# amirhajibabaei/AutoForce

Hardware: AMD Instinct MI355X
Metric: MD-step atoms*steps/sec (SGPR predict: NL + descriptors + K_nm + E/F/stress + covloss); `value`: a Langevin MD loop on the device, every step from the forces of the one before (sgpr_md_run; --steps dependent steps between two fences); `value_resident_frames`: steps over independent frames resident i (higher is better)
Workload: dtype f64

## Files before the change

### autoforce_amd/csrc/api.hip

```cpp
#include <math.h>
#include <stdarg.h>
#include <stdio.h>
#include <stdlib.h>
#include <string.h>

#include <algorithm>
#include <numeric>

#include <dlfcn.h>
#include <unistd.h>
#include <rccl/rccl.h>

#include "../../include/sgpr_hip.h"
#include "sgpr_internal.h"
#include <cmath>
#include <limits>

static thread_local char g_err[512] = "";
static int fail(int code, const char *fmt, ...)
{
    va_list ap;
    va_start(ap, fmt);
    vsnprintf(g_err, sizeof(g_err), fmt, ap);
    va_end(ap);
// ... 341 lines not shown
        const int r = r0 + k, c = c0 + threadIdx.x;
        t[k][threadIdx.x] = (r < rows && c < cols) ? A[(size_t)r * lda + c] : 0.0;
    }
    __syncthreads();
    for (int k = threadIdx.y; k < 32; k += blockDim.y) {
        const int c = c0 + k, r = r0 + threadIdx.x;
        if (c < cols && r < rows) B[(size_t)c * ldb + r] = t[threadIdx.x][k];
    }
}

#define SGPR_MD_SCAL 16
struct FinNext {
    int mode;
    int S, cap, force, step;
    int pbc[3];
    double thr2;
    const double *pos_in;
    const int *iperm, *cslot;
    double *pos;
    int *flags;
    int *bc_next, *bc_cur;
    int *bin_of, *kslot;
    BinRec *b_rec;
    BinAux *b_aux;
    double *csq_rw;
    const double *x_cur, *v_cur;
    double *x_next, *v_next;
    const double *mass, *sig;
    const double *noise;
    unsigned long long seed;
    long long t_index;
    double hdt, c1;
    int nh, nh_first;
    const double *x_prev;
    double *v_now;
    const double *nh_zeta;
    int pending;
    double *ke_cur;
    const double *ke_prev, *packed_prev;
    double ediff;
    int *halt;
    int *halt_host;
    double *scal_cur, *scal_prev;
    int *mark_cur;
};

struct FinArgs {
    int N, cnt, first, stride, maxnn, t_stride, has_beta, nE, nV, bin_cap, t_check, csq_slots;
    int nbins_clear;
    const int *perm, *slot, *nn, *nbr_j, *aux, *nn_raw;
    const unsigned short *T;
    const double *G;
    const double *Fnbr, *Fself;
    const double *csq, *vs_sqrt, *Epart, *virpart;
    double mean_energy;
    double *packed;
    int *stat, *bin_count;
    const int *row_cols, *row_colslot, *nbr_code;
    size_t g_stride, f_stride, v_stride, p_stride;
    int xp;
    int xcmax;
    size_t scal_off;
    const int *flag;
    int *rebuilds;
    const double *pos;
    double *pos0;
    const double *cell;
    const NlGrid *grid;
    double *cell0;
    FinNext nx;
};

template <int CTRL>
__device__ __forceinline__ double fin_dpp(double v)
{
    const int lo = __builtin_amdgcn_update_dpp(0, __double2loint(v), CTRL, 0xf, 0xf, true);
    const int hi = __builtin_amdgcn_update_dpp(0, __double2hiint(v), CTRL, 0xf, 0xf, true);
    return __hiloint2double(hi, lo);
}
__device__ __forceinline__ double fin_lane(double v, int l)
{
    return __hiloint2double(__builtin_amdgcn_readlane(__double2hiint(v), l), __builtin_amdgcn_readlane(__double2loint(v), l));
}
__device__ __forceinline__ double fin_wave_sum(double v)
{
    v += fin_dpp<0xB1>(v);
    v += fin_dpp<0x4E>(v);
    v += fin_dpp<0x141>(v);
    v += fin_dpp<0x140>(v);
    return (fin_lane(v, 0) + fin_lane(v, 16)) + (fin_lane(v, 32) + fin_lane(v, 48));
}

__device__ __forceinline__ void finalize_reduce(const FinArgs &f, int q)
{
    __shared__ double wsum[4];
    const int tid = threadIdx.x, wave = tid >> 6, lane = tid & 63;
    const size_t by = blockIdx.y;
    double s = 0.0;
    if (q == 10) {
        int m8[8] = {0, 0, 0, 0, 0, 0, 0, 0};
        const int4 *src4 = (const int4 *)f.nn_raw;
        const int n4 = (f.cnt + 3) / 4;
        for (int k0 = tid; k0 < n4; k0 += 1024) {
#pragma unroll
            for (int u = 0; u < 4; u++) {
                const int k = k0 + 256 * u;
                const int4 v = src4[min(k, n4 - 1)];
                const int e = 4 * k;
                int m = e < f.cnt ? v.x : 0;
                m = max(m, e + 1 < f.cnt ? v.y : 0);
                m = max(m, e + 2 < f.cnt ? v.z : 0);
                m = max(m, e + 3 < f.cnt ? v.w : 0);
                m8[u] = max(m8[u], m);
            }
        }
        const int mx = max(max(max(m8[0], m8[1]), max(m8[2], m8[3])), max(max(m8[4], m8[5]), max(m8[6], m8[7])));
        s = (double)mx;
#pragma unroll
        for (int o = 32; o > 0; o >>= 1) s = fmax(s, __shfl_xor(s, o, 64));
    } else {
        const double *src = q == 0 ? f.Epart : f.virpart + by * f.v_stride + (size_t)(q - 1) * f.nV;
        const int n = q == 0 ? f.nE : f.nV;
        double a8[8] = {0.0, 0.0, 0.0, 0.0, 0.0, 0.0, 0.0, 0.0};
        for (int k0 = tid; k0 < n; k0 += 2048) {
#pragma unroll
            for (int u = 0; u < 8; u++) {
                const int k = k0 + 256 * u;
                const double v = src[min(k, n - 1)];
                a8[u] += k < n ? v : 0.0;
            }
        }
        s = ((a8[0] + a8[1]) + (a8[2] + a8[3])) + ((a8[4] + a8[5]) + (a8[6] + a8[7]));
        s = fin_wave_sum(s);
    }
    if (lane == 0) wsum[wave] = s;
    __syncthreads();
    if (tid == 0) {
        if (q == 10 && by == 0) {
            if (*f.flag) {
                atomicAdd(f.rebuilds, 1);
                if (f.cell0 && f.cell) {
                    double cv[18];
#pragma unroll
                    for (int k = 0; k < 9; k++) { cv[k] = f.cell[k]; cv[9 + k] = f.grid->inv[k]; }
#pragma unroll
                    for (int k = 0; k < 18; k++) f.cell0[k] = cv[k];
                }
            }
            const int mx = (int)fmax(fmax(wsum[0], wsum[1]), fmax(wsum[2], wsum[3]));
            f.stat[0] = max(f.stat[0], mx);
            const bool ov = mx > f.maxnn || f.stat[1] > f.bin_cap || (f.t_check && f.stat[2] > f.t_stride) || f.stat[3] != 0;
            f.packed[f.scal_off + 10] = ov ? 1.0 : 0.0;
            if (f.nx.mode == 2) {
                f.nx.scal_cur[10] = ov ? 1.0 : 0.0;
                *f.nx.mark_cur = 1;
                if (ov) {
                    atomicMin(&f.nx.halt[0], f.nx.step);
                    f.nx.halt_host[1] = f.nx.step;
                }
            }
        } else if (q != 10) {
            const double v = ((wsum[0] + wsum[1]) + (wsum[2] + wsum[3])) + (q == 0 ? f.mean_energy : 0.0);
            f.packed[by * f.p_stride + f.scal_off + q] = v;
            if (f.nx.mode == 2) f.nx.scal_cur[q] = v;
        }
    }
}

__device__ __forceinline__ void finalize_reduce_prev(const FinArgs &f, int q)
{
    __shared__ double wprev[4], wprev2[4];
    const int tid = threadIdx.x, wave = tid >> 6, lane = tid & 63;
    const int N = f.N;
// ... 232 lines not shown
    if (lane < 3) packed[3 * (size_t)c + lane] = fs - (lane == 0 ? fx : lane == 1 ? fy : fz);
    if (lane < 3 && *f.flag) f.pos0[3 * (size_t)i + lane] = f.pos[3 * (size_t)i + lane];
    if (lane == 3) {
        const double v = 1.0 - cs;
        packed[3 * (size_t)f.N + c] = f.has_beta ? sqrt(v > 0.0 ? v : 0.0) * vs : 0.0;
    }
}

__device__ __forceinline__ double md_deviate(unsigned long long seed, long long t, int atom, int comp)
{
    unsigned c0 = (unsigned)t, c1 = (unsigned)((unsigned long long)t >> 32), c2 = (unsigned)atom, c3 = (unsigned)comp;
    unsigned k0 = (unsigned)seed, k1 = (unsigned)(seed >> 32);
#pragma unroll
    for (int r = 0; r < 10; r++) {
        const unsigned long long p0 = (unsigned long long)0xD2511F53u * c0, p1 = (unsigned long long)0xCD9E8D57u * c2;
        const unsigned n0 = (unsigned)(p1 >> 32) ^ c1 ^ k0, n1 = (unsigned)p1, n2 = (unsigned)(p0 >> 32) ^ c3 ^ k1, n3 = (unsigned)p0;
        c0 = n0; c1 = n1; c2 = n2; c3 = n3;
        k0 += 0x9E3779B9u; k1 += 0xBB67AE85u;
    }
    const unsigned long long a = ((unsigned long long)c0 << 32) | c1, b = ((unsigned long long)c2 << 32) | c3;
    const double u1 = (double)((a >> 11) + 1ull) * (1.0 / 9007199254740992.0);
    const double u2 = (double)(b >> 11) * (1.0 / 9007199254740992.0);
    return sqrt(-2.0 * log(u1)) * cos(6.283185307179586 * u2);
}

__global__ void md_deviates_kernel(int N, int rows, unsigned long long seed, long long t0, double *out)
{
    const size_t n3 = (size_t)3 * N, tot = n3 * rows;
    for (size_t e = (size_t)blockIdx.x * blockDim.x + threadIdx.x; e < tot; e += (size_t)gridDim.x * blockDim.x) {
        const size_t r = e / n3, w = e - r * n3;
        out[e] = md_deviate(seed, t0 + (long long)r, (int)(w / 3), (int)(w % 3));
    }
}

__device__ __forceinline__ double md_nh_advance(const FinNext &x, double F, double ms, double xc, double v0, double xprev, double zeta, double &xn)
{
#pragma clang fp contract(off)
    const double dt = 2.0 * x.hdt;
    const double a = __ddiv_rn((dt * dt) * F, ms);
    double xp = xprev;
    if (x.nh_first) xp = (xc - dt * v0) + 0.5 * a;
    const double b = x.hdt * zeta;
    const double num = ((2.0 * xc) - xp * (1.0 - b)) + a;
    xn = __ddiv_rn(num, 1.0 + b);
    return x.nh_first ? v0 : __ddiv_rn(xn - xp, 2.0 * dt);
}

__global__ __launch_bounds__(256) void md_nh_kernel(int N, const double *ke, double *zeta, int n, double dt, double c1, double c2, double K0,
                                                    const int *halt, int step, double *scal_row)
{
    if (*halt < step) return;
    __shared__ double wsum[4];
    const int tid = threadIdx.x;
    double s = 0.0;
    for (int k = tid; k < N; k += 256) s += ke[2 * (size_t)k];
    s = fin_wave_sum(s);
    if ((tid & 63) == 0) wsum[tid >> 6] = s;
    __syncthreads();
    if (tid == 0) {
#pragma clang fp contract(off)
        const double KE = 0.5 * ((wsum[0] + wsum[1]) + (wsum[2] + wsum[3]));
        const int sc = n & 3, sn = (n + 1) & 3, sp = (n + 3) & 3;
        const double d = KE - K0;
        const double zprev = n == 0 ? -(c1 * d) : zeta[sp];
        const double zcur = n == 0 ? 0.0 : zeta[sc];
        const double zint = n == 0 ? 0.0 : zeta[4 + sc];
        const double znew = zprev + c2 * d;
        zeta[sn] = znew;
        zeta[4 + sn] = zint + dt * znew;
        scal_row[14] = zcur;
        scal_row[15] = zint;
    }
}

template <int MODE>
__global__ __launch_bounds__(256) void finalize_next_kernel(FinArgs f)
{
    const int tid = threadIdx.x, b = blockIdx.x, nA = gridDim.x - 13;
    const FinNext &x = f.nx;
    const int halt_w = MODE == 2 ? *x.halt : 0x7fffffff;
    if (b >= nA) {
        if (halt_w < x.step) return;
        if (b >= nA + 11) {
            if (MODE == 2 && x.packed_prev) finalize_reduce_prev(f, b - nA - 11);
        } else
            finalize_reduce(f, b - nA);
        return;
    }
    const int s1 = x.step + 1;
    const int wave = __builtin_amdgcn_readfirstlane(tid >> 6), lane = tid & 63;
    const int i = b * 4 + wave;
    const bool act = i < f.N;
    const int ia = act ? i : 0;
    const int l3 = lane < 3 ? lane : 2, lg = lane < f.maxnn ? lane : f.maxnn - 1, lc = lane < f.csq_slots ? lane : f.csq_slots - 1;
    const int rebuilt = *f.flag;
    const NlGrid g = *f.grid;
    const double2 *grow = (const double2 *)(f.G + ((size_t)ia * f.maxnn + lg) * 4);
    double2 g0 = grow[0], g1 = grow[1];
    const int n_ld = f.nn[ia];
    double fs = f.Fself[3 * (size_t)ia + l3];
    const int c = f.perm[ia];
    const int slot_i = f.slot[ia];
    const int ib = MODE == 1 ? x.iperm[ia] : ia;
    const int slot_b = MODE == 1 ? x.cslot[ia] : slot_i;
    double xc = 0.0, p0 = 0.0, vc = 0.0, ms = 1.0, sg = 0.0, nz = 0.0, xn = 0.0;
    if (MODE == 1) xn = x.pos_in[3 * (size_t)ia + l3];
    if (MODE == 2) {
        xc = x.x_cur[3 * (size_t)ia + l3];
        p0 = f.pos0[3 * (size_t)ia + l3];
        vc = x.v_cur[3 * (size_t)ia + l3];
        ms = x.mass[ia];
        sg = x.sig[ia];
        nz = x.noise ? x.noise[3 * (size_t)ia + l3] : 0.0;
    }
    double xpv = 0.0, zeta = 0.0;
    if (MODE == 2 && x.nh) { xpv = x.x_prev[3 * (size_t)ia + l3]; zeta = *x.nh_zeta; }
    double csv = f.has_beta ? f.csq[(size_t)ia * f.csq_slots + lc] : 0.0;
    if (lane >= f.csq_slots) csv = 0.0;
    if (f.has_beta)
        for (int k = lane + 64; k < f.csq_slots; k += 64) csv += f.csq[(size_t)ia * f.csq_slots + k];
    if (lane >= f.maxnn) { g0 = make_double2(0.0, 0.0); g1 = g0; }
    if (lane >= 3) fs = 0.0;
    const int n = act ? n_ld : 0;
    const double vs = f.has_beta ? f.vs_sqrt[slot_i < x.S ? slot_i : 0] : 0.0;
    if (MODE == 1) {
        xc = x.pos[3 * (size_t)ib + l3];
        p0 = f.pos0[3 * (size_t)ib + l3];
    }
    if (halt_w < x.step) return;
    for (int k = b * 256 + tid; k < f.nbins_clear; k += nA * 256) x.bc_cur[(size_t)k * SGPR_BIN_STRIDE] = 0;
    if (b == 0 && tid == 0) {
        if (x.force) atomicMax(&x.flags[s1 & 3], 1);
        x.flags[(s1 + 2) & 3] = 0;
        fin_cell_guard(f, rebuilt, s1);
    }
    if (!act) return;
    if (f.has_beta)
        for (int k = lane; k < f.csq_slots; k += 64) x.csq_rw[(size_t)i * f.csq_slots + k] = 0.0;
    int bin = 0, kb = -1, w0 = 0, w1 = 0, w2 = 0;
    auto place = [&](double X, double Y, double Z) {
        int bidx[3], w[3];
#pragma unroll
        for (int k = 0; k < 3; k++) {
            double fr = X * g.inv[k] + Y * g.inv[3 + k] + Z * g.inv[6 + k];
            w[k] = 0;
            bidx[k] = 0;
            if (x.pbc[k] && (g.inv[k] != 0.0 || g.inv[3 + k] != 0.0 || g.inv[6 + k] != 0.0)) {
                const double fl = floor(fr);
                w[k] = (int)fl;
                fr -= fl;
                const int bb = (int)(fr * g.nb[k]);
                bidx[k] = bb >= g.nb[k] ? g.nb[k] - 1 : (bb < 0 ? 0 : bb);
            }
        }
        bin = (bidx[0] * g.nb[1] + bidx[1]) * g.nb[2] + bidx[2];
        w0 = w[0]; w1 = w[1]; w2 = w[2];
        if (slot_b < x.S) kb = atomicAdd(&x.bc_next[(size_t)bin * SGPR_BIN_STRIDE], 1);
    };
    double X = 0.0, Y = 0.0, Z = 0.0;
    if (MODE == 1) {
        X = fin_lane(xn, 0); Y = fin_lane(xn, 1); Z = fin_lane(xn, 2);
        if (lane == 0) place(X, Y, Z);
    }
    const double cs = f.has_beta ? fin_wave_sum(csv) : 1.0;
    double fx = 0.0, fy = 0.0, fz = 0.0;
    for (int t0 = 0; t0 < n; t0 += 64) {
        const int t = t0 + lane;
        if (t < n) {
            double2 b0 = g0, b1 = g1;
            if (t0 > 0) {
                const double2 *row = (const double2 *)(f.G + ((size_t)i * f.maxnn + t) * 4);
                b0 = row[0]; b1 = row[1];
            }
            fx += b0.x; fy += b0.y; fz += b1.x;
        }
    }
    fx = fin_wave_sum(fx); fy = fin_wave_sum(fy); fz = fin_wave_sum(fz);
    const double Fv = fs - (lane == 0 ? fx : lane == 1 ? fy : fz);
    if (lane < 3) f.packed[3 * (size_t)c + lane] = Fv;
    if (lane == 3) {
        const double v = 1.0 - cs;
        f.packed[3 * (size_t)f.N + c] = f.has_beta ? sqrt(v > 0.0 ? v : 0.0) * vs : 0.0;
    }
    double ke = 0.0, kp = 0.0;
    if (MODE == 2 && x.nh) {
        if (lane < 3) {
            const double vnow = md_nh_advance(x, Fv, ms, xc, vc, xpv, zeta, xn);
            ke = ms * (vnow * vnow);
            kp = ke;
            x.x_next[3 * (size_t)i + lane] = xn;
            x.v_now[3 * (size_t)i + lane] = vnow;
        }
    } else if (MODE == 2 && lane < 3) {
#pragma clang fp contract(off)
        const double kick = __ddiv_rn(x.hdt * Fv, ms);
        double v = vc;
        if (x.pending) v = v + kick;
        ke = ms * (v * v);
        kp = ms * (vc * vc);
        const double v2 = v + kick;
        const double x1 = xc + x.hdt * v2;
        if (!x.noise && x.seed != 0ull && sg != 0.0) nz = md_deviate(x.seed, x.t_index, c, lane);
        const double v3 = x.c1 * v2 + sg * nz;
        xn = x1 + x.hdt * v3;
        x.x_next[3 * (size_t)i + lane] = xn;
        x.v_next[3 * (size_t)i + lane] = v3;
    }
    if (MODE == 2) {
        const double k3 = fin_lane(ke, 0) + fin_lane(ke, 1) + fin_lane(ke, 2);
        const double p3 = fin_lane(kp, 0) + fin_lane(kp, 1) + fin_lane(kp, 2);
        if (lane == 0) *(double2 *)(x.ke_cur + 2 * (size_t)i) = make_double2(k3, p3);
        X = fin_lane(xn, 0); Y = fin_lane(xn, 1); Z = fin_lane(xn, 2);
        if (lane == 0) place(X, Y, Z);
    }
    if (rebuilt) p0 = xc;
    if (lane < 3) {
        x.pos[3 * (size_t)ib + lane] = xn;
        if (rebuilt) f.pos0[3 * (size_t)ib + lane] = xc;
    }
    const double dd = xn - p0;
    const double d2 = fin_lane(dd, 0) * fin_lane(dd, 0) + fin_lane(dd, 1) * fin_lane(dd, 1) + fin_lane(dd, 2) * fin_lane(dd, 2);
    if (lane == 0) {
        if (!(d2 <= x.thr2)) atomicMax(&x.flags[s1 & 3], 1);
        x.bin_of[ib] = bin;
        x.kslot[ib] = kb;
        if (slot_b < x.S) {
            if (max(max(abs(w0), abs(w1)), abs(w2)) > 32767) atomicMax(&f.stat[3], 1);
            if (kb < x.cap) {
                const size_t e = (size_t)bin * x.cap + kb;
                BinRec r;
                r.x = X; r.y = Y; r.z = Z; r.idx = ib; r.pad = 0;
                x.b_rec[e] = r;
                BinAux ax;
                ax.w0 = (short)w0; ax.w1 = (short)w1; ax.w2 = (short)w2; ax.slot = (short)slot_b;
                x.b_aux[e] = ax;
            } else
                atomicMax(&f.stat[1], kb + 1);
        }
    }
}

__global__ void md_sort_rows_kernel(int N, int rows, const int *perm, const double *in, double *out)
{
    const size_t n3 = (size_t)3 * N, tot = n3 * rows;
    for (size_t e = (size_t)blockIdx.x * blockDim.x + threadIdx.x; e < tot; e += (size_t)gridDim.x * blockDim.x) {
        const size_t r = e / n3, w = e - r * n3;
        const int i = (int)(w / 3), k = (int)(w - 3 * (size_t)i);
        out[e] = in[r * n3 + 3 * (size_t)perm[i] + k];
    }
}

__global__ __launch_bounds__(256) void finalize_tail_kernel(FinArgs f)
{
    if (*f.nx.halt < f.nx.step) return;
    finalize_reduce_prev(f, (int)blockIdx.x);
}

void host_build_harm_coef(HarmCoef *hc)
{
    memset(hc, 0, sizeof(*hc));
    hc->y00 = sqrt(1.0 / (4.0 * M_PI));
    for (int l = 2; l <= SGPR_MAX_L; l++)
        for (int m = 0; m < l - 1; m++) {
            hc->al[l][m] = sqrt((4.0 * l * l - 1.0) / (l * l - m * m));
            hc->bl[l][m] = -sqrt(((l - 1.0) * (l - 1.0) - m * m) / (4.0 * (l - 1.0) * (l - 1.0) - 1.0));
        }
    for (int l = 0; l <= SGPR_MAX_L; l++) hc->cl[l] = sqrt(2.0 * l + 1.0);
    for (int l = 1; l <= SGPR_MAX_L; l++) hc->dl[l] = -sqrt(1.0 + 1.0 / (2.0 * l));
}

static double factorial(int n)
{
    double f = 1.0;
    for (int i = 2; i <= n; i++) f *= i;
    return f;
}

static void build_pack(sgpr_model *h)
{
    const int N1 = h->nmax + 1, L1 = h->lmax + 1, U = h->S * N1;
    h->D = N1 * N1 * L1;
    h->Dc = U * (U + 1) / 2 * L1;
    h->Dpad = rup(h->Dc, 32);
    h->CS = h->S * N1 * L1 * L1;
    h->h_pack.assign(h->Dc, PackEntry());
    for (int u = 0; u < U; u++)
        for (int v = u; v < U; v++)
            for (int l = 0; l < L1; l++) {
                const int pair = u * U - (u * (u - 1)) / 2 + (v - u);
                PackEntry &e = h->h_pack[pair * L1 + l];
                const int n1 = u % N1, n2 = v % N1;
                const double a1 = 1.0 / ((2 * l + 1) * pow(2.0, 2 * n1 + l) * factorial(n1) * factorial(n1 + l));
                const double a2 = 1.0 / ((2 * l + 1) * pow(2.0, 2 * n2 + l) * factorial(n2) * factorial(n2 + l));
                e.u = (int16_t)u; e.v = (int16_t)v; e.l = (int16_t)l; e.pad = 0;
                e.coef = sqrt(a1 * a2) * (u == v ? 1.0 : 1.4142135623730951);
            }
}

static int slot_of(const sgpr_model *h, int z)
{
    for (int k = 0; k < h->S; k++)
        if (h->species[k] == z) return k;
    return -1;
}

extern "C" const char *sgpr_last_error(void) { return g_err; }
extern "C" int sgpr_version(void) { return 1000; }

extern "C" int sgpr_device_count(void)
{
    int n = 0;
    if (hipGetDeviceCount(&n) != hipSuccess) return 0;
    return n;
}

extern "C" int sgpr_create(int lmax, int nmax, double eta, double rc, int S, const int32_t *species_z,
                           const double *radii, int device, sgpr_model **out)
{
    if (!out || !species_z || S < 1 || S > SGPR_MAX_S) return fail(SGPR_E_INVALID, "sgpr_create: bad species table (S=%d)", S);
    if (!(rc > 0.0) || !(eta > 0.0)) return fail(SGPR_E_INVALID, "sgpr_create: rc and eta must be positive");
    const bool in234 = lmax >= 2 && lmax <= 4 && nmax >= 2 && nmax <= 4;
    const bool ok = in234 && (S <= 8 || (lmax == 3 && nmax == 3));
// ... 864 lines not shown
        std::copy(h->slot_sorted.begin(), h->slot_sorted.end(), ss.begin());
        HIPCHK(hipMemcpy(h->d_slot.p, ss.data(), sizeof(int) * h->N_rows, hipMemcpyHostToDevice));
    }
    HIPCHK(hipMemcpy(h->d_aoff.p, h->aoff.data(), sizeof(int) * (h->S + 1), hipMemcpyHostToDevice));
    HIPCHK(hipMemcpy(h->d_lslot.p, lslot.data(), sizeof(int) * h->cnt_rows, hipMemcpyHostToDevice));
    HIPCHK(hipMemcpy(h->d_lnn.p, lnn.data(), sizeof(int) * h->cnt_rows, hipMemcpyHostToDevice));
    h->maxnn = 0;
    h->d_nbr_j.release();
    h->d_nbr_shift.release();
    h->d_T.release();
    h->t_stride = 0;
    h->gather_ok = !h->force_scatter;
    h->warm = false;
    h->bind_gen++;
    return alloc_work(h);
}

extern "C" int64_t sgpr_packed_len(int N) { return 4 * (int64_t)N + 11; }

#include "peer.inc"

static void stamp(sgpr_model *h, const char *name, hipStream_t st)
{
    if (!h->profile) return;
    const size_t k = h->stage_names.size();
    if (h->ev.size() <= k + 1) {
        while (h->ev.size() <= k + 1) {
            hipEvent_t e;
            (void)hipEventCreate(&e);
            h->ev.push_back(e);
        }
    }
    h->stage_names.push_back(name);
    (void)hipEventRecord(h->ev[k + 1], st);
}

struct FinBatch { int batch; double *G, *F, *virpart; size_t g_stride, f_stride, v_stride, p_stride; const int *cols; };

struct StepNext {
    int mode = 0;
    const double *pos_next = nullptr;
    FinNext md;
};

static void launch_finalize(sgpr_model *h, bool gather, int nE, int nV, bool beta, double mean_energy,
                            double *packed_dev, hipStream_t st, const FinBatch *fb = nullptr, const StepNext *nx = nullptr,
                            unsigned step = 0, bool xp = false, const ShardSrc *consume = nullptr)
{
    const int N = h->N;
    FinArgs f = {};
    f.xp = xp ? 1 : 0; f.xcmax = (int)peer_cmax(N, h->world);
    f.scal_off = xp ? 3 * (size_t)N + 4 * (size_t)f.xcmax : 4 * (size_t)N;
    f.N = N; f.cnt = h->cnt; f.first = h->rank; f.stride = h->world; f.maxnn = h->maxnn; f.t_stride = h->t_stride;
    f.has_beta = beta ? 1 : 0; f.nE = nE; f.nV = nV; f.bin_cap = h->bin_cap; f.nbins_clear = 4096;
    f.t_check = (h->world == 1 && h->gather_ok) ? 1 : 0;
    f.perm = h->d_perm.p; f.slot = h->d_slot.p; f.nn = h->d_nn.p; f.nbr_j = h->d_nbr_j.p; f.aux = h->d_aux.p;
    f.nn_raw = h->d_nn_raw.p; f.T = h->d_T.p; f.G = h->d_G.p; f.Fnbr = h->d_F.p; f.Fself = h->d_F.p + 3 * (size_t)N;
    f.csq = h->d_csq.p; f.csq_slots = h->csq_slots; f.vs_sqrt = h->d_vs_sqrt.p; f.Epart = h->d_Epart.p; f.virpart = h->d_virpart.p;
    f.mean_energy = mean_energy; f.packed = packed_dev; f.stat = h->d_stat.p; f.bin_count = h->d_bin_count.p;
    f.flag = h->step_flag ? h->step_flag : h->d_flag.p; f.pos = h->d_pos.p; f.pos0 = h->d_pos0.p;
    f.rebuilds = h->d_flag.p + 4;
    f.cell = h->last_cell; f.grid = (const NlGrid *)h->d_grid.p; f.cell0 = h->d_cell0.p;
    int batch = 1;
    if (fb) step = h->step_count - 1;
    if (fb) {
        f.flag = h->d_flag.p + 5;
        batch = fb->batch;
        f.G = fb->G; f.Fnbr = fb->F; f.Fself = fb->F + 3 * (size_t)N; f.virpart = fb->virpart;
        f.g_stride = fb->g_stride; f.f_stride = fb->f_stride; f.v_stride = fb->v_stride; f.p_stride = fb->p_stride;
        f.row_cols = fb->cols; f.row_colslot = h->d_ind_slot.p; f.nbr_code = h->d_nbr_shift.p;
    }
    f.bin_count = h->d_bin_count.p + SGPR_BIN_INTS * (step & 1u);
    if (nx && nx->mode) {
        FinNext &x = f.nx;
        if (nx->mode == 2) x = nx->md;
        x.mode = nx->mode; x.S = h->S; x.cap = h->bin_cap; x.force = h->skin <= 0.0 ? 1 : 0; x.step = (int)step;
        for (int k = 0; k < 3; k++) x.pbc[k] = h->pbc[k];
        x.thr2 = 0.25 * h->skin * h->skin;
        x.pos_in = nx->pos_next; x.pos = h->d_pos.p; x.flags = h->d_flag.p;
        x.iperm = h->d_perm.p + N; x.cslot = h->d_perm.p + 2 * (size_t)N;
        x.bc_cur = h->d_bin_count.p + SGPR_BIN_INTS * (step & 1u); x.bc_next = h->d_bin_count.p + SGPR_BIN_INTS * ((step + 1) & 1u);
        x.bin_of = h->d_bin_of.p; x.kslot = h->d_kslot.p; x.b_rec = h->d_b_rec.p; x.b_aux = h->d_b_aux.p;
        x.csq_rw = h->d_csq.p;
        const dim3 grid((std::max(N, 1) + 3) / 4 + 13);
        if (consume) {
            const dim3 gs((std::max(N, 1) + 63) / 64 + 3);
            if (nx->mode == 1) hipLaunchKernelGGL(shard_next_kernel<1>, gs, dim3(256), 0, st, f, *consume);
            else hipLaunchKernelGGL(shard_next_kernel<2>, gs, dim3(256), 0, st, f, *consume);
            return;
        }
        if (!gather) {
            x.csq_rw = h->d_csq.p;
            hipLaunchKernelGGL(finalize_scatter_next_kernel, dim3((std::max(N, 1) + 255) / 256 + 11), dim3(256), 0, st, f);
        } else if (nx->mode == 1) hipLaunchKernelGGL(finalize_next_kernel<1>, grid, dim3(256), 0, st, f);
        else hipLaunchKernelGGL(finalize_next_kernel<2>, grid, dim3(256), 0, st, f);
        return;
    }
    if (gather)
        hipLaunchKernelGGL(finalize_gather_kernel, dim3((std::max(N, 1) + 3) / 4 + 11, batch), dim3(256), 0, st, f);
    else
        hipLaunchKernelGGL(finalize_kernel, dim3((std::max(N, 1) + 255) / 256 + 11, batch), dim3(256), 0, st, f);
}

static int enqueue_step(sgpr_model *h, const double *pos_dev, const double *cell_dev, double *packed_dev,
                        hipStream_t st, const StepNext *nx = nullptr, bool no_exchange = false)
{
    const int N = h->N, cnt = h->cnt;
    h->last_cell = cell_dev;
    if (h->profile) {
        h->stage_names.clear();
        if (h->ev.empty()) {
            hipEvent_t e;
            (void)hipEventCreate(&e);
            h->ev.push_back(e);
        }
        (void)hipEventRecord(h->ev[0], st);
    }
    NlParams np = {};
    np.N = N; np.S = h->S;
    for (int k = 0; k < 3; k++) np.pbc[k] = h->pbc[k];
    const bool gather = h->world == 1 && h->gather_ok && h->d_T.p != nullptr;
    NlScratch sc = {(NlGrid *)h->d_grid.p, h->d_bin_of.p, h->d_kslot.p, h->d_bin_count.p, h->bin_cap, h->d_b_rec.p,
                    h->d_b_aux.p, h->d_slot.p, h->d_stat.p, h->d_nn_raw.p, h->d_aux.p, gather ? h->d_T.p : nullptr,
                    h->t_stride};
    const double skin = h->use_graph ? 0.0 : h->skin;
    const unsigned step = h->step_count++;
    sc.bin_count = h->d_bin_count.p + SGPR_BIN_INTS * (step & 1u);
    sc.flag = h->d_flag.p; sc.parity = (int)(step & 1u); sc.fslot = (int)(step & 3u); sc.fclear = (int)((step + 2) & 3u);
    sc.force = (!h->lists_valid || skin <= 0.0) ? 1 : 0;
    sc.skin = skin; sc.pos0 = h->d_pos0.p; sc.cell0 = h->d_cell0.p; sc.ncand = h->d_ncand.p; sc.cand_j = h->d_cand_j.p;
    sc.cand_code = h->d_cand_code.p; sc.cidx = h->d_cidx.p; sc.hm = h->d_hm.p; sc.hmw = h->hmw;
    h->step_flag = h->d_flag.p + sc.fslot;
    const bool pre = h->pre_valid && h->pre_pos == pos_dev && h->pre_cell == cell_dev && h->pre_step == step && !sc.force;
    if (h->pre_valid && !pre) (void)hipMemsetAsync(sc.bin_count, 0, SGPR_BIN_INTS * sizeof(int), st);
    h->pre_valid = false;
    if (!pre) {
        launch_neighbor_bin(np, h->bin_identity ? nullptr : h->d_perm.p, pos_dev, h->d_pos.p, cell_dev, h->rc + skin, sc, h->d_F.p, 3 * N,
                            h->d_csq.p, cnt * h->csq_slots, st);
        stamp(h, "neighbor_bin", st);
    }
    DescParams dp = {};
    dp.lmax = h->lmax; dp.nmax = h->nmax; dp.S = h->S; dp.N = cnt; dp.Nall = N; dp.first = h->rank;
    dp.stride = h->world; dp.maxnn = h->maxnn; dp.Dc = h->Dc; dp.Dpad = h->Dpad; dp.CS = h->CS; dp.rc = h->rc;
    for (int k = 0; k < SGPR_MAX_S; k++) dp.radii_v[k] = k < h->S ? h->radii[k] : 1.0;
    if (h->d_stamps.p && h->d_pstamps.n < (size_t)16 * N) h->d_pstamps.alloc((size_t)16 * N);
    dp.stamps = h->d_stamps.p ? h->d_pstamps.p : nullptr;
    dp.xq = h->xcd_quads ? h->gemm_bm_k / 4 : 0;
    dp.stat = h->d_stat.p;
    int rcd = launch_list_forward(dp, sc, h->d_pos.p, cell_dev, h->d_pack.p, h->d_nn.p, h->d_lnn.p, h->d_nbr_j.p,
                                  h->d_nbr_shift.p, h->d_Pn.p, h->d_norm.p, h->d_C.p, h->d_shear.p, h->d_prec.p, st);
    if (rcd) return fail(SGPR_E_UNSUPPORTED, "descriptor kernel not compiled in");
    stamp(h, "list_forward", st);
    const bool predict = h->m > 0 && h->has_mu && cnt > 0 && !h->rows_mu;
    const bool beta = h->m > 0 && h->has_choli && cnt > 0 && !h->rows_mu;
    const bool cov_rev = h->cov_in_rev && h->gemm_bm_w == 32 && h->gemm_kd_w == 16 && h->t_covl.n > 0 && SGPR_REV_WPW(h->S) == 4;
    const bool fused3 = predict && beta && h->gemm_fused && h->t_fused.n > 0 && !h->use_graph &&
                        !(h->use_fork && h->side && !h->profile) && !cov_rev;
    if (h->m > 0 && cnt > 0 && !fused3) {
        gemm_kernel_pm(h, h->d_Pn.p, cnt, h->d_lslot.p, h->d_lnn.p, h->t_knm, h->d_K.p, h->d_Aw.p,
                       h->rows_mu ? h->rows_mu : (h->has_mu ? h->d_mu.p : nullptr), h->d_Epart.p, st);
        stamp(h, "gemm_knm", st);
    }
    GemmParams gw = {}, gc = {};
    gw.M = cnt; gw.N = h->Dpad; gw.K = h->m_pad;
    gw.lda = h->m_pad; gw.ldb = h->m_pad; gw.ldc = h->Dpad;
    gw.A = h->d_Aw.p; gw.B = h->d_PmT.p; gw.C = h->d_W.p;
    gw.tiles = h->t_w.p; gw.ntiles = (int)h->t_w.n; gw.bm = h->gemm_bm_w; gw.kd = h->gemm_kd_w;
// ... 1064 lines not shown
```

Measured before the change: 46.17 million.

## Map one atom per 16-lane row in finalize_next kernel

The fused finalize/next-step kernel now gives each atom a 16-lane row instead of a whole 64-lane wave, so one block handles 16 atoms rather than 4. Each lane loads four neighbour gradient rows, and the row reductions use DPP row operations without cross-row readlanes. Component broadcasts use quad-permute DPP. The bin clearing is moved to the end of the kernel, and the flag and cell-guard setup is moved into an extra tail block. This is meant to reduce wasted lanes and launched blocks when neighbour counts are small. The cost is more registers per lane and reliance on row-local DPP correctness.

Result: faster. 47.04 million (median of 6 runs) (+1.9%).

```diff
diff --git a/autoforce_amd/csrc/api.hip b/autoforce_amd/csrc/api.hip
--- a/autoforce_amd/csrc/api.hip
+++ b/autoforce_amd/csrc/api.hip
@@ -447,13 +447,27 @@
 {
     return __hiloint2double(__builtin_amdgcn_readlane(__double2hiint(v), l), __builtin_amdgcn_readlane(__double2loint(v), l));
 }
-__device__ __forceinline__ double fin_wave_sum(double v)
+__device__ __forceinline__ double fin_row_sum(double v)
 {
     v += fin_dpp<0xB1>(v);
     v += fin_dpp<0x4E>(v);
     v += fin_dpp<0x141>(v);
     v += fin_dpp<0x140>(v);
+    return v;
+}
+__device__ __forceinline__ double fin_wave_sum(double v)
+{
+    v = fin_row_sum(v);
     return (fin_lane(v, 0) + fin_lane(v, 16)) + (fin_lane(v, 32) + fin_lane(v, 48));
+}
+__device__ __forceinline__ double fin_row_sum4(const double (&v)[4])
+{
+    return (fin_row_sum(v[0]) + fin_row_sum(v[1])) + (fin_row_sum(v[2]) + fin_row_sum(v[3]));
+}
+template <int K>
+__device__ __forceinline__ double fin_quad_lane(double v)
+{
+    return fin_dpp<K * 0x55>(v);
 }
 
 __device__ __forceinline__ void finalize_reduce(const FinArgs &f, int q)
@@ -852,25 +866,38 @@
     if (b >= nA) {
         if (halt_w < x.step) return;
         if (b >= nA + 11) {
+            if (b == nA + 12 && tid == 0) {
+                const int s1 = x.step + 1;
+                if (x.force) atomicMax(&x.flags[s1 & 3], 1);
+                x.flags[(s1 + 2) & 3] = 0;
+                fin_cell_guard(f, *f.flag, s1);
+            }
             if (MODE == 2 && x.packed_prev) finalize_reduce_prev(f, b - nA - 11);
         } else
             finalize_reduce(f, b - nA);
         return;
     }
     const int s1 = x.step + 1;
-    const int wave = __builtin_amdgcn_readfirstlane(tid >> 6), lane = tid & 63;
-    const int i = b * 4 + wave;
+    const int lane = tid & 15;
+    const int i = b * 16 + (tid >> 4);
     const bool act = i < f.N;
     const int ia = act ? i : 0;
-    const int l3 = lane < 3 ? lane : 2, lg = lane < f.maxnn ? lane : f.maxnn - 1, lc = lane < f.csq_slots ? lane : f.csq_slots - 1;
+    const int l3 = lane < 3 ? lane : 2;
+    const int c = f.perm[ia];
+    const int slot_i = f.slot[ia];
     const int rebuilt = *f.flag;
     const NlGrid g = *f.grid;
-    const double2 *grow = (const double2 *)(f.G + ((size_t)ia * f.maxnn + lg) * 4);
-    double2 g0 = grow[0], g1 = grow[1];
     const int n_ld = f.nn[ia];
+    double2 g0[4];
+    double g1[4];
+#pragma unroll
+    for (int j = 0; j < 4; j++) {
+        const int s = lane + 16 * j;
+        const double *p = f.G + ((size_t)ia * f.maxnn + (s < f.maxnn ? s : f.maxnn - 1)) * 4;
+        g0[j] = *(const double2 *)p;
+        g1[j] = p[2];
+    }
     double fs = f.Fself[3 * (size_t)ia + l3];
-    const int c = f.perm[ia];
-    const int slot_i = f.slot[ia];
     const int ib = MODE == 1 ? x.iperm[ia] : ia;
     const int slot_b = MODE == 1 ? x.cslot[ia] : slot_i;
     double xc = 0.0, p0 = 0.0, vc = 0.0, ms = 1.0, sg = 0.0, nz = 0.0, xn = 0.0;
@@ -885,28 +912,35 @@
     }
     double xpv = 0.0, zeta = 0.0;
     if (MODE == 2 && x.nh) { xpv = x.x_prev[3 * (size_t)ia + l3]; zeta = *x.nh_zeta; }
-    double csv = f.has_beta ? f.csq[(size_t)ia * f.csq_slots + lc] : 0.0;
-    if (lane >= f.csq_slots) csv = 0.0;
+    const double *cqp = f.has_beta ? f.csq + (size_t)ia * f.csq_slots : f.Fself;
+    double cq[4];
+#pragma unroll
+    for (int j = 0; j < 4; j++) {
+        const int s = lane + 16 * j;
+        cq[j] = cqp[f.has_beta && s < f.csq_slots ? s : (f.has_beta ? f.csq_slots - 1 : 0)];
+        if (!f.has_beta || s >= f.csq_slots) cq[j] = 0.0;
+    }
     if (f.has_beta)
-        for (int k = lane + 64; k < f.csq_slots; k += 64) csv += f.csq[(size_t)ia * f.csq_slots + k];
-    if (lane >= f.maxnn) { g0 = make_double2(0.0, 0.0); g1 = g0; }
-    if (lane >= 3) fs = 0.0;
-    const int n = act ? n_ld : 0;
+#pragma unroll
+        for (int j = 0; j < 4; j++)
+            for (int k = lane + 16 * j + 64; k < f.csq_slots; k += 64) cq[j] += f.csq[(size_t)ia * f.csq_slots + k];
     const double vs = f.has_beta ? f.vs_sqrt[slot_i < x.S ? slot_i : 0] : 0.0;
     if (MODE == 1) {
         xc = x.pos[3 * (size_t)ib + l3];
         p0 = f.pos0[3 * (size_t)ib + l3];
     }
+#pragma unroll
+    for (int j = 0; j < 4; j++)
+        if (lane + 16 * j >= f.maxnn) { g0[j] = make_double2(0.0, 0.0); g1[j] = 0.0; }
+    if (lane >= 3) fs = 0.0;
+    const int n = act ? n_ld : 0;
     if (halt_w < x.step) return;
-    for (int k = b * 256 + tid; k < f.nbins_clear; k += nA * 256) x.bc_cur[(size_t)k * SGPR_BIN_STRIDE] = 0;
-    if (b == 0 && tid == 0) {
-        if (x.force) atomicMax(&x.flags[s1 & 3], 1);
-        x.flags[(s1 + 2) & 3] = 0;
-        fin_cell_guard(f, rebuilt, s1);
-    }
-    if (!act) return;
+    auto clear_bins = [&]() {
+        for (int k = b * 256 + tid; k < f.nbins_clear; k += nA * 256) x.bc_cur[(size_t)k * SGPR_BIN_STRIDE] = 0;
+    };
+    if (!act) { clear_bins(); return; }
     if (f.has_beta)
-        for (int k = lane; k < f.csq_slots; k += 64) x.csq_rw[(size_t)i * f.csq_slots + k] = 0.0;
+        for (int k = lane; k < f.csq_slots; k += 16) x.csq_rw[(size_t)i * f.csq_slots + k] = 0.0;
     int bin = 0, kb = -1, w0 = 0, w1 = 0, w2 = 0;
     auto place = [&](double X, double Y, double Z) {
         int bidx[3], w[3];
@@ -929,24 +963,37 @@
     };
     double X = 0.0, Y = 0.0, Z = 0.0;
     if (MODE == 1) {
-        X = fin_lane(xn, 0); Y = fin_lane(xn, 1); Z = fin_lane(xn, 2);
+        X = fin_quad_lane<0>(xn); Y = fin_quad_lane<1>(xn); Z = fin_quad_lane<2>(xn);
         if (lane == 0) place(X, Y, Z);
     }
-    const double cs = f.has_beta ? fin_wave_sum(csv) : 1.0;
-    double fx = 0.0, fy = 0.0, fz = 0.0;
-    for (int t0 = 0; t0 < n; t0 += 64) {
-        const int t = t0 + lane;
-        if (t < n) {
-            double2 b0 = g0, b1 = g1;
-            if (t0 > 0) {
-                const double2 *row = (const double2 *)(f.G + ((size_t)i * f.maxnn + t) * 4);
-                b0 = row[0]; b1 = row[1];
+    double cs = 1.0;
+    if (f.has_beta) {
+        cs = fin_row_sum4(cq);
+        __builtin_amdgcn_sched_barrier(0);
+    }
+    double fx[4], fy[4], fz[4];
+#pragma unroll
+    for (int j = 0; j < 4; j++) {
+        fx[j] = 0.0; fy[j] = 0.0; fz[j] = 0.0;
+        if (lane + 16 * j < n) { fx[j] += g0[j].x; fy[j] += g0[j].y; fz[j] += g1[j]; }
+    }
+    for (int t0 = 64; t0 < n; t0 += 64) {
+#pragma unroll
+        for (int j = 0; j < 4; j++) {
+            const int t = t0 + lane + 16 * j;
+            if (t < n) {
+                const double *row = f.G + ((size_t)i * f.maxnn + t) * 4;
+                const double2 b0 = *(const double2 *)row;
+                fx[j] += b0.x; fy[j] += b0.y; fz[j] += row[2];
             }
-            fx += b0.x; fy += b0.y; fz += b1.x;
-        }
-    }
-    fx = fin_wave_sum(fx); fy = fin_wave_sum(fy); fz = fin_wave_sum(fz);
-    const double Fv = fs - (lane == 0 ? fx : lane == 1 ? fy : fz);
+        }
+    }
+    const double Fx = fin_row_sum4(fx);
+    __builtin_amdgcn_sched_barrier(0);
+    const double Fy = fin_row_sum4(fy);
+    __builtin_amdgcn_sched_barrier(0);
+    const double Fz = fin_row_sum4(fz);
+    const double Fv = fs - (lane == 0 ? Fx : lane == 1 ? Fy : Fz);
     if (lane < 3) f.packed[3 * (size_t)c + lane] = Fv;
     if (lane == 3) {
         const double v = 1.0 - cs;
@@ -977,10 +1024,10 @@
         x.v_next[3 * (size_t)i + lane] = v3;
     }
     if (MODE == 2) {
-        const double k3 = fin_lane(ke, 0) + fin_lane(ke, 1) + fin_lane(ke, 2);
-        const double p3 = fin_lane(kp, 0) + fin_lane(kp, 1) + fin_lane(kp, 2);
+        const double k3 = fin_quad_lane<0>(ke) + fin_quad_lane<1>(ke) + fin_quad_lane<2>(ke);
+        const double p3 = fin_quad_lane<0>(kp) + fin_quad_lane<1>(kp) + fin_quad_lane<2>(kp);
         if (lane == 0) *(double2 *)(x.ke_cur + 2 * (size_t)i) = make_double2(k3, p3);
-        X = fin_lane(xn, 0); Y = fin_lane(xn, 1); Z = fin_lane(xn, 2);
+        X = fin_quad_lane<0>(xn); Y = fin_quad_lane<1>(xn); Z = fin_quad_lane<2>(xn);
         if (lane == 0) place(X, Y, Z);
     }
     if (rebuilt) p0 = xc;
@@ -989,7 +1036,8 @@
         if (rebuilt) f.pos0[3 * (size_t)ib + lane] = xc;
     }
     const double dd = xn - p0;
-    const double d2 = fin_lane(dd, 0) * fin_lane(dd, 0) + fin_lane(dd, 1) * fin_lane(dd, 1) + fin_lane(dd, 2) * fin_lane(dd, 2);
+    const double dx = fin_quad_lane<0>(dd), dy = fin_quad_lane<1>(dd), dz = fin_quad_lane<2>(dd);
+    const double d2 = dx * dx + dy * dy + dz * dz;
     if (lane == 0) {
         if (!(d2 <= x.thr2)) atomicMax(&x.flags[s1 & 3], 1);
         x.bin_of[ib] = bin;
@@ -1008,6 +1056,7 @@
                 atomicMax(&f.stat[1], kb + 1);
         }
     }
+    clear_bins();
 }
 
 __global__ void md_sort_rows_kernel(int N, int rows, const int *perm, const double *in, double *out)
@@ -2038,7 +2087,7 @@
         x.bc_cur = h->d_bin_count.p + SGPR_BIN_INTS * (step & 1u); x.bc_next = h->d_bin_count.p + SGPR_BIN_INTS * ((step + 1) & 1u);
         x.bin_of = h->d_bin_of.p; x.kslot = h->d_kslot.p; x.b_rec = h->d_b_rec.p; x.b_aux = h->d_b_aux.p;
         x.csq_rw = h->d_csq.p;
-        const dim3 grid((std::max(N, 1) + 3) / 4 + 13);
+        const dim3 grid((std::max(N, 1) + 15) / 16 + 13);
         if (consume) {
             const dim3 gs((std::max(N, 1) + 63) / 64 + 3);
             if (nx->mode == 1) hipLaunchKernelGGL(shard_next_kernel<1>, gs, dim3(256), 0, st, f, *consume);
```
